# kfkq/DQMC

Hardware: AMD Instinct MI355X
Metric: MC sweeps/sec, 2D Hubbard N=256 Ltau=200 (higher is better)
Workload: dtype f64; 1 GPU; cfg3: 16x16 Hubbard U=8.0 beta=8.0 Ltau=200 n_stab=10 t=1 mu=-0.1; chains_per_gpu=1, n_chains_total=1, parallelism=independent chains, 1 gpu x 1 chain

## Files before the change

dqmc_amd/csrc/common.h:

```cpp
#pragma once

#include <hip/hip_runtime.h>
#include <cstdint>
#include <memory>
#include <string>

struct dqmc_engine;

namespace dq {

constexpr int WAVE = 64;

void set_error(const std::string& msg);
const char* get_error();

#define DQ_HIP(call)                                                                    \
    do {                                                                                \
        hipError_t _e = (call);                                                         \
        if (_e != hipSuccess) {                                                         \
            ::dq::set_error(std::string(#call) + ": " + hipGetErrorString(_e));         \
            return -2;                                              \
        }                                                                               \
    } while (0)

// ... 58 lines not shown
int launch_transpose_scale(CMat in, Mat out, CVec rs, int n, int n_chains, hipStream_t s);
int launch_max_abs_diff(CMat A, CMat B, double* err, long err_stride, int n, int n_chains, hipStream_t s);
int launch_add_scaled_cols(CMat A, CMat B, CVec cs, Mat C, int n, int n_chains, hipStream_t s);
int launch_scale_rows(CMat in, CVec rs, Mat out, int n, int n_chains, hipStream_t s);
struct DevStats { double acc_rate, max_err, sum_err, n_err; long long n_accepted, n_proposed; };
int launch_fold_stats(DevStats* st, const int* acc, long acc_stride, int n_slices, const double* err, long err_stride, int n_err,
                      int n, int nt, int n_chains, hipStream_t s);

struct QrWork {
    double* tau; long tau_stride;
    int* jpvt; long jpvt_stride;
    unsigned long long* sync = nullptr; long sync_stride = 0;
    int* abort_words = nullptr;
    int* info = nullptr;
    double* pw = nullptr; long pw_stride = 0;
    bool pw_two_launch = false;
    int* pivpos = nullptr; long pivpos_stride = 0;
};
bool qr_panel_fused_fits(int n);
bool qr_panel_fused_default(int n);
long qr_panel_work_doubles(int n, bool two_launch);
int launch_qr_panel(Mat A, Mat L, QrWork w, int n, int n_chains, hipStream_t s);
long qrcp_coop_sync_granules(int n);
int qrcp_coop_workgroups(int n, int n_chains);
enum class QrFamily { Panel, ColumnOwner, Cooperative, Streaming };
int launch_to_ldr(QrFamily f, Mat A, Mat L, Vec d, Mat R, QrWork w, int n, int n_chains, hipStream_t s);

int launch_lu_blocked(Mat A, int* perm, long perm_stride, int* rowpos, long rowpos_stride, double* logabsdet, int accumulate_logdet,
                      int* info, int n, int n_chains, hipStream_t s);
int launch_lu_solve(CMat LU, const int* perm, long perm_stride, Mat X, CVec dg, int mode, int n, int n_chains, hipStream_t s);

int launch_tri_solve(CMat R, const int* perm, long perm_stride, Mat X, CVec dg, double* scratch, long scratch_stride, int n, int n_chains, hipStream_t s);

int launch_gj_solve(Mat A, Mat B, Mat X, Mat SA, double* tinv, int* perm, long perm_stride, int* rowpos, long rowpos_stride,
                    double* logabsdet, int accumulate_logdet, int* info, int n, int n_chains, hipStream_t s);

struct UpdateTables {
    double rb[4][3];
    double delta[4][3];
    double ev[4];
    double iev[4];
    double pad[32];
};
struct UpdateDesc {
    Mat G;
    int8_t* fields; long f_stride;
    double* expv; double* invexpv; long v_stride;
    const UpdateTables* tabs;
    const int32_t* perm; const uint8_t* kprop; const double* u; long rs_stride;
    double* Upanel; double* Wpanel; long panel_stride;
    double* Cpanel = nullptr;
    int* state; long state_stride;
    double* prep; long prep_stride;
    Mat GT{nullptr, 0};
    int gt_valid = 0;
    void* slice_sync = nullptr;
    unsigned slice_epoch = 0;
    int slice_absent_tile = -1;
    int slice_absent_l = -1;
    int slice_late_tile = -1, slice_late_us = 0;
    int* info = nullptr;
    int* acc_out; long acc_stride;
    int n, nt;
};
constexpr int UPDATE_KD = 32;

struct SliceSync {
    unsigned long long seq; unsigned int error; unsigned int solo_count; unsigned int pad[12];
// ... 42 lines not shown
```

dqmc_amd/csrc/engine.hip:

```cpp
#include "common.h"
#include "../../include/dqmc_hip.h"

#include <cmath>
#include <cstdlib>
#include <cstring>
#include <map>
#include <memory>
#include <mutex>
#include <vector>

namespace dq {

static thread_local std::string g_err;
void set_error(const std::string& msg) { g_err = msg; }
const char* get_error() { return g_err.c_str(); }

int init_device_kernels(int device) {
    static std::mutex mu; static bool done[64] = {};
    std::lock_guard<std::mutex> lk(mu);
    if (device < 0 || device >= 64) { set_error("device ordinal out of range"); return -1; }
    if (done[device]) return 0;
    DQ_HIP(hipSetDevice(device));
    DQ_TRY(update_init_device()); DQ_TRY(update_sm_init_device()); DQ_TRY(qr_init_device()); DQ_TRY(qr_colown_init_device());
    done[device] = true;
    return 0;
}

struct Switches { bool qr_panel; int qr_panel_fused; bool qr_streaming, walk_submatrix, lu_classic, slice_multikernel; };
static const Switches& switches() {
    static const Switches sw = [] {
        const char* panel = getenv("DQMC_QR_PANEL");
        const char* fused = getenv("DQMC_QR_PANEL_FUSED");
        return Switches{!(panel && atoi(panel) == 0), fused ? (atoi(fused) != 0 ? 1 : 0) : -1, getenv("DQMC_QR_STREAMING") != nullptr, getenv("DQMC_WALK_SUBMATRIX") != nullptr,
                        getenv("DQMC_LU_CLASSIC") != nullptr, getenv("DQMC_SLICE_MULTIKERNEL") != nullptr};
    }();
    return sw;
}

constexpr int GJ_MAX_N = 1024, GJ_MAX_CHAINS = 8;
constexpr int TRI_MAX_N = 640;

static QrFamily pick_qr(int n, int chains, bool allow_panel) {
    const Switches& sw = switches();
    if (sw.qr_streaming) return QrFamily::Streaming;
    if (allow_panel && sw.qr_panel && n >= 64 && n <= 1024 && n % 16 == 0 && chains <= 8) return QrFamily::Panel;
    if (n <= 256) return QrFamily::ColumnOwner;
    return qrcp_coop_workgroups(n, chains) <= 200 ? QrFamily::Cooperative : QrFamily::Streaming;
}

struct KernelPlan {
    QrFamily qr;
    enum class Solve { GaussJordan, BlockedLu } solve;
    enum class Rinv { Blocked, PerColumn } rinv;
    static KernelPlan pick(int n, int chains) {
        return KernelPlan{pick_qr(n, chains, true),
                          n <= GJ_MAX_N && chains <= GJ_MAX_CHAINS && !switches().lu_classic ? Solve::GaussJordan : Solve::BlockedLu,
                          n <= TRI_MAX_N ? Rinv::Blocked : Rinv::PerColumn};
    }
};

static SlicePath pick_slice_path(int n, int chains, bool reserved) {
    const Switches& sw = switches();
    const bool walk = n <= 256;
    if (sw.slice_multikernel) return SlicePath::Pairs;
    if (reserved) return walk && !sw.walk_submatrix ? SlicePath::PersistentWalk : SlicePath::PersistentSubmatrix;
    if (!walk) return SlicePath::Pairs;
// ... 14 lines not shown
    DevPtr<double> L, d, R, X;
    DevPtr<int> jpvt;
    std::unique_ptr<bool[]> tri, xok;
    int alloc(int k, int n_, int C_, bool with_x = false) {
        n = n_; C = C_;
        const size_t nn = (size_t)n * n;
        DQ_TRY(dev_alloc(L, (size_t)k * C * nn)); DQ_TRY(dev_alloc(d, (size_t)k * C * n));
        DQ_TRY(dev_alloc(R, (size_t)k * C * nn)); DQ_TRY(dev_alloc(jpvt, (size_t)k * C * n));
        if (with_x) DQ_TRY(dev_alloc(X, (size_t)k * C * nn));
        tri.reset(new bool[k]()); xok.reset(new bool[k]());
        return 0;
    }
    LdrRef at(int i) const {
        const long nn = (long)n * n;
        LdrRef f{Mat{L.get() + (long)i * C * nn, nn}, Vec{d.get() + (long)i * C * n, (long)n}, Mat{R.get() + (long)i * C * nn, nn},
                 jpvt.get() + (long)i * C * n, &tri[i]};
        if (X) { f.X = Mat{X.get() + (long)i * C * nn, nn}; f.xok = &xok[i]; }
        return f;
    }
};

struct Ctx {
    int n = 0, C = 0, device = 0;
    long nn = 0;
    hipStream_t stream = nullptr;
    static constexpr int NT = 6, NV = 5;
    DevPtr<double> pool;
    DevPtr<double> vpool;
    DevPtr<int> ipool;
    DevPtr<unsigned long long> qsync;
    DevPtr<int> qabort;
    DevPtr<double> tinv;
    DevPtr<double> qpw;
    bool qpw_two_launch = false;
    DevPtr<int> qpivpos;
    DevPtr<double> trinv;
    KernelPlan plan{};

    Mat T(int k) const { return Mat{pool.get() + (long)k * C * nn, nn}; }
    Vec V(int k) const { return Vec{vpool.get() + (long)k * C * n, (long)n}; }
    int* jpvt() const { return ipool.get(); }
    int* lperm() const { return ipool.get() + (long)C * n; }
    int* rowpos() const { return ipool.get() + 2L * C * n; }
    int* info() const { return ipool.get() + 3L * C * n; }

    int init(int n_, int C_, int device_) {
        n = n_; C = C_; device = device_; nn = (long)n * n;
        DQ_HIP(hipSetDevice(device));
        DQ_TRY(init_device_kernels(device));
        DQ_HIP(hipStreamCreateWithFlags(&stream, hipStreamNonBlocking));
        DQ_TRY(dev_alloc(pool, (size_t)NT * C * nn));
        DQ_TRY(dev_alloc(vpool, (size_t)NV * C * n));
        DQ_TRY(dev_alloc(ipool, 3L * C * n + 4));
        plan = KernelPlan::pick(n, C);
        if (plan.qr == QrFamily::Cooperative) { DQ_TRY(dev_alloc(qsync, (size_t)qrcp_coop_sync_granules(n) * C)); DQ_TRY(dev_alloc(qabort, C)); }
        if (plan.qr == QrFamily::Panel) {
            const int fused = switches().qr_panel_fused;
            qpw_two_launch = !(fused < 0 ? qr_panel_fused_default(n) : fused == 1 && qr_panel_fused_fits(n));
            const size_t qpw_count = (size_t)qr_panel_work_doubles(n, qpw_two_launch) * C;
            DQ_TRY(dev_alloc(qpw, qpw_count)); DQ_TRY(dev_alloc(qpivpos, (size_t)n * C));
            DQ_HIP(hipMemsetAsync(qpw.get(), 0, sizeof(double) * qpw_count, stream));
        }
        if (plan.solve == KernelPlan::Solve::GaussJordan) DQ_TRY(dev_alloc(tinv, (size_t)2048 * C));
        if (plan.rinv == KernelPlan::Rinv::Blocked) DQ_TRY(dev_alloc(trinv, (size_t)16 * (n + 16) * C));
        DQ_HIP(hipMemsetAsync(ipool.get(), 0, sizeof(int) * (3L * C * n + 4), stream));
        return 0;
    }
    ~Ctx() { if (stream) (void)hipStreamDestroy(stream); }

    int gemm(CMat A, CMat B, Mat Cm, CVec rs = CVec(), CVec ks = CVec(), CVec cs = CVec(), int transA = 0, int accumulate = 0, Mat CT = Mat{nullptr, 0}) {
        GemmDesc g; g.A = A; g.B = B; g.C = Cm; g.CT = CT; g.rs = rs; g.ks = ks; g.cs = cs; g.n = n; g.transA = transA; g.accumulate = accumulate;
        return launch_gemm(g, C, stream);
    }
    int to_ldr(Mat A, LdrRef out, bool direct = true) {
        const bool keep = direct && out.jpvt != nullptr;
        QrWork w{V(4).p, (long)n, keep ? out.jpvt : jpvt(), (long)n};
        w.sync = qsync.get(); w.sync_stride = qrcp_coop_sync_granules(n); w.abort_words = qabort.get(); w.info = info();
        w.pw = qpw.get(); w.pw_stride = qr_panel_work_doubles(n, qpw_two_launch); w.pw_two_launch = qpw_two_launch; w.pivpos = qpivpos.get(); w.pivpos_stride = n;
        if (out.tri) *out.tri = keep;
        out.touch();
        return launch_to_ldr(plan.qr, A, out.L, out.d, out.R, w, n, C, stream);
    }
    int r_inverse_scaled(LdrRef F, CVec dinv, Mat scratch, Mat lu_scratch, Mat* Xout) {
        const Mat X = F.X.p ? F.X : scratch;
        *Xout = X;
        if (F.xok && *F.xok) return 0;
        if (F.tri && *F.tri && F.jpvt) {
            if (plan.rinv == KernelPlan::Rinv::Blocked) DQ_TRY(launch_tri_solve(F.R, F.jpvt, n, X, dinv, trinv.get(), 16L * (n + 16), n, C, stream));
            else DQ_TRY(launch_lu_solve(F.R, F.jpvt, n, X, dinv, 2, n, C, stream));
        } else {
            DQ_TRY(launch_copy(F.R, lu_scratch, nn, C, stream));
            DQ_TRY(launch_lu_blocked(lu_scratch, lperm(), n, rowpos(), n, nullptr, 0, info(), n, C, stream));
            DQ_TRY(launch_lu_solve(lu_scratch, lperm(), n, X, dinv, 1, n, C, stream));
        }
        if (F.xok) *F.xok = true;
        return 0;
    }
    int mat_mul_ldr(CMat M, LdrRef F, LdrRef out) {
        DQ_TRY(gemm(M, F.L, T(0), CVec(), CVec(), CVec(F.d)));
        LdrRef q{out.L, out.d, T(1)};
        DQ_TRY(to_ldr(T(0), q));
        if (out.tri) *out.tri = false;
        out.touch();
        return gemm(T(1), F.R, out.R);
    }
    int ldr_mul_mat(LdrRef F, CMat M, LdrRef out) {
        DQ_TRY(gemm(F.R, M, T(0), CVec(F.d)));
        LdrRef q{T(1), out.d, out.R, out.jpvt, out.tri};
        q.xok = out.xok;
        DQ_TRY(to_ldr(T(0), q));
        return gemm(F.L, T(1), out.L);
    }
    int ldr_mul_ldr(LdrRef F1, LdrRef F2, LdrRef out) {
        DQ_TRY(gemm(F1.R, F2.L, T(0), CVec(F1.d), CVec(), CVec(F2.d)));
        LdrRef q{T(1), out.d, T(2)};
        DQ_TRY(to_ldr(T(0), q));
        if (out.tri) *out.tri = false;
        out.touch();
        DQ_TRY(gemm(F1.L, T(1), out.L));
        return gemm(T(2), F2.R, out.R);
    }
    int solve(Mat M, Mat RHS, Mat out, double* logdet_acc, Mat* Y) {
        if (plan.solve == KernelPlan::Solve::GaussJordan) {
            DQ_TRY(launch_gj_solve(M, RHS, out, T(5), tinv.get(), lperm(), n, rowpos(), n, logdet_acc, 1, info(), n, C, stream));
            *Y = out; return 0;
        }
        DQ_TRY(launch_lu_blocked(M, lperm(), n, rowpos(), n, logdet_acc, 1, info(), n, C, stream));
        DQ_TRY(launch_lu_solve(M, lperm(), n, RHS, CVec(), 0, n, C, stream));
        *Y = RHS; return 0;
    }
    int inv_I_plus_ldr(LdrRef F, Mat G, double* logdet ) {
        DQ_TRY(launch_split_d(F.d, V(0), V(1), logdet, n, C, stream));
        Mat X; DQ_TRY(r_inverse_scaled(F, V(0), T(1), T(0), &X));
        DQ_TRY(launch_add_scaled_cols(X, F.L, V(1), T(2), n, C, stream));
        DQ_TRY(launch_transpose_scale(T(2), T(3), CVec(), n, C, stream));
        DQ_TRY(launch_transpose_scale(X, T(4), CVec(), n, C, stream));
        Mat Y; DQ_TRY(solve(T(3), T(4), T(0), logdet, &Y));
        return launch_transpose_scale(Y, G, CVec(), n, C, stream);
    }
    int inv_I_plus_ldr_mul_ldr(LdrRef F1, LdrRef F2, Mat G, Mat GT = Mat{nullptr, 0}) {
        DQ_TRY(launch_split_d2(F1.d, V(0), V(1), F2.d, V(2), V(3), n, C, stream));
        Mat X; DQ_TRY(r_inverse_scaled(F2, V(2), T(1), T(0), &X));
        DQ_TRY(gemm(F1.L, X, T(2), V(0), CVec(), CVec(), 1));
        DQ_TRY(gemm(F1.R, F2.L, T(2), V(1), CVec(), V(3), 0, 1));
        DQ_TRY(launch_transpose_scale(F1.L, T(3), V(0), n, C, stream));
        Mat Y; DQ_TRY(solve(T(2), T(3), T(0), nullptr, &Y));
        return gemm(X, Y, G, CVec(), CVec(), CVec(), 0, 0, GT);
    }
    int inv_invldr_plus_ldr(LdrRef F1, LdrRef F2, Mat G, bool negate) {
        DQ_TRY(launch_split_d(F1.d, V(0), V(1), nullptr, n, C, stream));
        DQ_TRY(launch_split_d(F2.d, V(2), V(3), nullptr, n, C, stream));
        Mat X; DQ_TRY(r_inverse_scaled(F2, V(2), T(1), T(0), &X));
        DQ_TRY(gemm(F1.L, X, T(2), V(0), CVec(), CVec(), 1));
        DQ_TRY(gemm(F1.R, F2.L, T(2), V(1), CVec(), V(3), 0, 1));
        DQ_TRY(launch_scale_rows(F1.R, V(1), T(3), n, C, stream));
        Mat Y; DQ_TRY(solve(T(2), T(3), T(0), nullptr, &Y));
        DQ_TRY(gemm(X, Y, G));
// ... 946 lines not shown
```

dqmc_amd/csrc/lu_gj.hip:

```cpp
#include "common.h"
#include "wave.h"
#include <cstdlib>
#include <utility>

namespace dq {

namespace {
constexpr int GJ_NB = 32;
using d4 = __attribute__((ext_vector_type(4))) double;

__device__ __forceinline__ void lds_wait() { asm volatile("s_waitcnt lgkmcnt(0)" ::: "memory"); }

template <int NR, int J>
__device__ __forceinline__ void gj_step(double (&a)[NR][GJ_NB], bool (&live)[NR], int (&mypos)[NR], int& myperm, bool& singular, int lane, int k0) {
    unsigned long long best = 0ULL; int bq = -1;
#pragma unroll
    for (int q = 0; q < NR; ++q) {
        const unsigned long long kq = live[q] ? ((unsigned long long)__double_as_longlong(fabs(a[q][J])) | 1ULL) : 0ULL;
        if (kq > best) { best = kq; bq = q; }
    }
    const unsigned hi = (unsigned)(best >> 32), lo = (unsigned)best;
    const unsigned m1 = wave_max_u32(hi);
    const unsigned m2 = wave_max_u32(hi == m1 ? lo : 0u);
    const unsigned long long winners = __ballot(hi == m1 && lo == m2 && bq >= 0);
// ... 108 lines not shown
            const double s = s0 + s1;
            x[j] = up ? s / T0[sg * (j * 33)] : s;
        }
        double* out = tinv + GJ_NB * GJ_NB + 256 * blk + 16 * c;
#pragma unroll
        for (int j = 0; j < 16; ++j) out[up ? 15 - j : j] = x[j];
    }
}

__device__ __forceinline__ void gj_panel_logdet(double (&LU)[GJ_NB][GJ_NB], double* logabsdet, int accumulate, int* info, int chain, int lane, int nbw, int k0, int s_sing) {
    const double pv = lane < nbw ? fabs(LU[lane][lane]) : 1.0;
    const double ls = wave_sum(log(pv));
    if (lane == 0) {
        if (logabsdet) logabsdet[chain] = ((accumulate || k0 > 0) ? logabsdet[chain] : 0.0) + ls;
        if (info && (s_sing || !(ls == ls))) atomicOr(info, DQ_STATUS_PIVOT);
    }
}
template <int... Js>
__device__ __forceinline__ void gj_tri_steps(double (&x)[16], const double* T0, int sg, int cc, bool up, bool hi, double rd, std::integer_sequence<int, Js...>) {
    auto step = [&](auto jc) {
        constexpr int j = decltype(jc)::value;
        double s0 = (j == cc) ? 1.0 : 0.0, s1 = 0.0;
#pragma unroll
        for (int m = 0; m < j; ++m) {
            const double tt = T0[sg * (j * 32 + m)];
            if (m & 1) s1 = fma(-tt, x[m], s1); else s0 = fma(-tt, x[m], s0);
        }
        const double s = s0 + s1;
        const double r0 = readlane_f64(rd, 15 - j), r1 = readlane_f64(rd, 31 - j);
        x[j] = up ? s * (hi ? r1 : r0) : s;
    };
    (step(std::integral_constant<int, Js>{}), ...);
}
__device__ __forceinline__ void gj_panel_tri_inverses(double (&LU)[GJ_NB][GJ_NB], double* tinv, int lane) {
    const int blk = lane >> 4, c = lane & 15;
    const bool up = blk >= 2;
    const int base = (blk & 1) * 16;
    const double* T0 = &LU[0][0] + (up ? (base + 15) * 33 : base * 33);
    const int sg = up ? -1 : 1;
    const int cc = up ? 15 - c : c;
    const double rd = 1.0 / LU[lane & 31][lane & 31];
    double x[16];
    gj_tri_steps(x, T0, sg, cc, up, (blk & 1) != 0, rd, std::make_integer_sequence<int, 16>{});
    double* out = tinv + GJ_NB * GJ_NB + 256 * blk + 16 * c;
#pragma unroll
    for (int j = 0; j < 16; ++j) out[up ? 15 - j : j] = x[j];
}

#ifdef DQ_GJ_STAMPS
#define GST(i) { unsigned long long t_; asm volatile("s_waitcnt lgkmcnt(0)\n\ts_memtime %0\n\ts_waitcnt lgkmcnt(0)" : "=s"(t_) :: "memory"); gst[i] += t_ - gprev; gprev = t_; }
#define GST_ARGS , unsigned long long (&gst)[8], unsigned long long& gprev
#define GST_PASS , gst, gprev
#else
#define GST(i)
#define GST_ARGS
#define GST_PASS
#endif
template <int J, int NW, int RPL>
__device__ __forceinline__ void gj_step_mw(double (&a)[RPL][GJ_NB], unsigned& live, int (&mypos)[RPL], int& myperm, bool& singular, int lane, int wave, int k0,
                                           double (*slot_row)[NW][GJ_NB + 2], unsigned long long (*slot_key)[(NW + 1) & ~1] GST_ARGS) {
    constexpr int PAR = J & 1;
    constexpr int C0 = J & ~1;
    GST(0)
    double aj = a[0][J]; int bs = 0;
    if (RPL > 1) asm volatile("" : "+v"(aj));
    unsigned long long key = (live & 1u) ? ((unsigned long long)__double_as_longlong(fabs(aj)) | 1ULL) : 0ULL;
#pragma unroll
    for (int q = 1; q < RPL; ++q) {
        double v = a[q][J];
        asm volatile("" : "+v"(v));
        const unsigned long long kq = ((live >> q) & 1u) ? ((unsigned long long)__double_as_longlong(fabs(v)) | 1ULL) : 0ULL;
        if (kq > key) { key = kq; aj = v; bs = q; }
    }
    double rme = __builtin_amdgcn_rcp(aj);
    rme = fma(fma(-aj, rme, 1.0), rme, rme);
    rme = fma(fma(-aj, rme, 1.0), rme, rme);
    const unsigned hi = (unsigned)(key >> 32), lo = (unsigned)key;
// ... 34 lines not shown
    double prow[GJ_NB - C0];
#pragma unroll
    for (int c = C0; c < GJ_NB; c += 2) { const double2 v = *reinterpret_cast<const double2*>(&slot_row[PAR][pw][c]); prow[c - C0] = v.x; prow[c + 1 - C0] = v.y; }
    const double r = slot_row[PAR][pw][GJ_NB];
    GST(5)
    if (lane == J && wave == 0) myperm = pl + 64 * pw + 64 * NW * ps;
    const bool mine = wave == pw && lane == pl;
    singular = singular || !(fabs(prow[J - C0]) > 0.0);
#pragma unroll
    for (int q = 0; q < RPL; ++q) {
        if (mine && ps == q) { live &= ~(1u << q); mypos[q] = k0 + J; }
        const bool lv = (live >> q) & 1u;
        const double l = lv ? a[q][J] * r : 0.0;
        a[q][J] = lv ? l : a[q][J];
#pragma unroll
        for (int c = J + 1; c < GJ_NB; ++c) a[q][c] = fma(-l, prow[c - C0], a[q][c]);
    }
    GST(6)
}
template <int J, int NW, int RPL>
struct GjStepsMW {
    static __device__ __forceinline__ void run(double (&a)[RPL][GJ_NB], unsigned& live, int (&mypos)[RPL], int& myperm, bool& singular, int lane, int wave, int nbw, int k0,
                                               double (*slot_row)[NW][GJ_NB + 2], unsigned long long (*slot_key)[(NW + 1) & ~1] GST_ARGS) {
        if (J < nbw) gj_step_mw<J, NW, RPL>(a, live, mypos, myperm, singular, lane, wave, k0, slot_row, slot_key GST_PASS);
        GjStepsMW<J + 1, NW, RPL>::run(a, live, mypos, myperm, singular, lane, wave, nbw, k0, slot_row, slot_key GST_PASS);
    }
};
template <int NW, int RPL>
struct GjStepsMW<GJ_NB, NW, RPL> {
    static __device__ __forceinline__ void run(double (&)[RPL][GJ_NB], unsigned&, int (&)[RPL], int&, bool&, int, int, int, int, double (*)[NW][GJ_NB + 2],
                                               unsigned long long (*)[(NW + 1) & ~1] GST_ARGS) {}
};
template <int NW, int RPL>
__global__ __launch_bounds__(64 * NW) void gj_panel_mw_kernel(CMat Am, int* rowpos_p, long rowpos_stride, int* perm_p, long perm_stride, double* tinv_p,
                                                          double* logabsdet, int accumulate, int* info, int n, int k0) {
    constexpr int NWK = (NW + 1) & ~1;
    __shared__ __attribute__((aligned(16))) double LU[GJ_NB][GJ_NB];
    __shared__ __attribute__((aligned(16))) double slot_row[2][NW][GJ_NB + 2];
    __shared__ __attribute__((aligned(16))) unsigned long long slot_key[2][NWK];
    __shared__ int s_sing;
    static_assert(RPL <= 4, "two key bits name the slot");
    const int chain = blockIdx.y;
    const double* __restrict__ A = Am.at(chain);
    int* rowpos = rowpos_p + (long)chain * rowpos_stride;
    int* perm = perm_p + (long)chain * perm_stride;
    double* tinv = tinv_p + (long)chain * 2 * GJ_NB * GJ_NB;
    const int t = threadIdx.x, lane = t & 63, wave = t >> 6;
#ifdef DQ_GJ_STAMPS
    unsigned long long gentry;
    asm volatile("s_memtime %0\n\ts_waitcnt lgkmcnt(0)" : "=s"(gentry) :: "memory");
#endif
    const int nbw = min(GJ_NB, n - k0);
    unsigned live = 0u;
    int mypos[RPL], myperm = 0; bool singular = false;
    double a[RPL][GJ_NB];
#pragma unroll
    for (int q = 0; q < RPL; ++q) {
        const int r = t + 64 * NW * q;
        const bool lv = r < n && (k0 == 0 ? true : rowpos[r < n ? r : 0] < 0);
        live |= lv ? (1u << q) : 0u;
        mypos[q] = -1;
#pragma unroll
        for (int c = 0; c < GJ_NB; ++c) a[q][c] = (lv && c < nbw) ? A[r + (long)n * (k0 + c)] : 0.0;
    }
    for (int e = t; e < GJ_NB * GJ_NB; e += blockDim.x) (&LU[0][0])[e] = ((e >> 5) == (e & 31)) ? 1.0 : 0.0;
    if (t == 0) s_sing = 0;
    if (t < 2 * NWK) (&slot_key[0][0])[t] = 0ULL;
    __syncthreads();

#ifdef DQ_GJ_STAMPS
    unsigned long long gst[8] = {0, 0, 0, 0, 0, 0, 0, 0}, gprev, gstart;
    asm volatile("s_waitcnt vmcnt(0)\n\ts_memtime %0\n\ts_waitcnt lgkmcnt(0)" : "=s"(gprev) :: "memory"); gstart = gprev;
#endif
    GjStepsMW<0, NW, RPL>::run(a, live, mypos, myperm, singular, lane, wave, nbw, k0, slot_row, slot_key GST_PASS);
#ifdef DQ_GJ_STAMPS
    if (t == 0 && k0 == 0 && blockIdx.y == 0)
        printf("gj panel k0=0 n=%d, %d waves x %d rows per lane, clocks over %d steps (each segment includes one stamp, ~130): (loop) %llu | search %llu | publish %llu | barrier %llu | keys %llu | row %llu | fma %llu | total %llu\n",
               n, (int)(blockDim.x >> 6), RPL, nbw, gst[0], gst[1], gst[2], gst[3], gst[4], gst[5], gst[6], gprev - gstart);
#endif

    __syncthreads();
#pragma unroll
    for (int q = 0; q < RPL; ++q) {
        const int r = t + 64 * NW * q;
        if (r < n) { if (k0 == 0) rowpos[r] = mypos[q]; else if (mypos[q] >= 0) rowpos[r] = mypos[q]; }
        if (mypos[q] >= 0) {
            double* dst = &LU[mypos[q] - k0][0];
#pragma unroll
            for (int c = 0; c < GJ_NB; c += 2) *reinterpret_cast<double2*>(dst + c) = make_double2(a[q][c], a[q][c + 1]);
        }
    }
    if (wave == 0 && lane < nbw) perm[k0 + lane] = myperm;
    if (singular && lane == 0) s_sing = 1;
    __syncthreads();
    for (int e = t; e < GJ_NB * GJ_NB; e += blockDim.x) tinv[e] = (&LU[0][0])[e];
#ifdef DQ_GJ_STAMPS
    unsigned long long gmid;
    asm volatile("s_waitcnt vmcnt(0)\n\ts_memtime %0\n\ts_waitcnt lgkmcnt(0)" : "=s"(gmid) :: "memory");
#endif
    if (wave == 0) gj_panel_tri_inverses(LU, tinv, lane);
    else if (wave == 1) gj_panel_logdet(LU, logabsdet, accumulate, info, chain, lane, nbw, k0, s_sing);
#ifdef DQ_GJ_STAMPS
    unsigned long long gend;
    asm volatile("s_waitcnt vmcnt(0)\n\ts_memtime %0\n\ts_waitcnt lgkmcnt(0)" : "=s"(gend) :: "memory");
    if (t == 0 && k0 == 0 && blockIdx.y == 0) printf("   prologue %llu | steps %llu | LU hand-over (+ printf) %llu | epilogue %llu\n", gstart - gentry, gprev - gstart, gmid - gprev, gend - gmid);
#endif
}

__global__ __launch_bounds__(256) void gj_update_kernel(Mat Am, Mat Bm, Mat SAm, Mat Xm, const int* rowpos_p, long rowpos_stride,
                                                        const int* perm_p, long perm_stride, const double* tinv_p, int n, int k0, int nA, int nS, int nCA) {
    const int chain = blockIdx.y;
    double* __restrict__ A = Am.at(chain);
    double* __restrict__ B = Bm.at(chain);
    double* __restrict__ SA = SAm.at(chain);
    double* __restrict__ X = Xm.at(chain);
    const int* rowpos = rowpos_p + (long)chain * rowpos_stride;
    const int* perm = perm_p + (long)chain * perm_stride;
    const double* __restrict__ LUg = tinv_p + (long)chain * 2 * GJ_NB * GJ_NB;
    const double* __restrict__ Tinv = LUg + GJ_NB * GJ_NB;
    const int nbw = min(GJ_NB, n - k0);
    const int row_tiles = nA + nS + 1;
    const int rt = blockIdx.x % row_tiles, ct = blockIdx.x / row_tiles;
    const int lane = threadIdx.x & 63, wave = threadIdx.x >> 6;
    const int r16 = lane & 15, kk = lane >> 4;
    const int wr = wave & 1, wc = wave >> 1;
    const bool colA = ct < nCA;
    const int col = (colA ? k0 + nbw + 32 * ct : 32 * (ct - nCA)) + 16 * wc + r16;
    const bool col_ok = col < n;
    const long coff = (long)n * (col_ok ? col : n - 1);
    const double* __restrict__ src12 = colA ? A : B;
    double* __restrict__ dstS = colA ? SA : X;

    double a12[2][4];
#pragma unroll
    for (int h = 0; h < 2; ++h)
#pragma unroll
        for (int s = 0; s < 4; ++s) {
// ... 46 lines not shown
    d4 w = {a12[1][0], a12[1][1], a12[1][2], a12[1][3]};
#pragma unroll
    for (int s = 0; s < 4; ++s) w = __builtin_amdgcn_mfma_f64_16x16x4f64(cl[s], t1[0][s], w, 0, 0, 0);
    t1[1] = zero4;
#pragma unroll
    for (int s = 0; s < 4; ++s) t1[1] = __builtin_amdgcn_mfma_f64_16x16x4f64(lbi[s], w[s], t1[1], 0, 0, 0);
    u[1] = zero4;
#pragma unroll
    for (int s = 0; s < 4; ++s) u[1] = __builtin_amdgcn_mfma_f64_16x16x4f64(ubi[s], t1[1][s], u[1], 0, 0, 0);
    w = t1[0];
#pragma unroll
    for (int s = 0; s < 4; ++s) w = __builtin_amdgcn_mfma_f64_16x16x4f64(cu[s], u[1][s], w, 0, 0, 0);
    u[0] = zero4;
#pragma unroll
    for (int s = 0; s < 4; ++s) u[0] = __builtin_amdgcn_mfma_f64_16x16x4f64(uai[s], w[s], u[0], 0, 0, 0);
    if (writer) {
#pragma unroll
        for (int reg = 0; reg < 4; ++reg) {
            const int i = 16 * wr + kk + 4 * reg;
            if (i < nbw && col_ok) dstS[k0 + i + coff] = u[wr][reg];
        }
        return;
    }
    d4 acc = {0.0, 0.0, 0.0, 0.0};
#pragma unroll
    for (int h = 0; h < 2; ++h)
#pragma unroll
        for (int s = 0; s < 4; ++s) acc = __builtin_amdgcn_mfma_f64_16x16x4f64(mult[h][s], u[h][s], acc, 0, 0, 0);
#pragma unroll
    for (int reg = 0; reg < 4; ++reg)
        if (st_ok[reg]) dst[row0 + kk + 4 * reg + coff] = cold[reg] - acc[reg];
}

int launch_gj_solve(Mat A, Mat B, Mat X, Mat SA, double* tinv, int* perm, long perm_stride, int* rowpos, long rowpos_stride,
                    double* logabsdet, int accumulate_logdet, int* info, int n, int n_chains, hipStream_t s) {
    if (n > 1024) { set_error("gj_solve supports n <= 1024"); return -1; }
    for (int k0 = 0; k0 < n; k0 += GJ_NB) {
        const dim3 pg(1, n_chains);
#define DQ_GJ_PANEL(NW, RPL) hipLaunchKernelGGL((gj_panel_mw_kernel<NW, RPL>), pg, dim3(RPL == 1 ? 64 * ((n + 63) / 64) : 64 * NW), 0, s, CMat(A), rowpos, rowpos_stride, perm, perm_stride, tinv, logabsdet, accumulate_logdet, info, n, k0)
        if (n > 768) DQ_GJ_PANEL(8, 2);
        else if (n > 576) DQ_GJ_PANEL(4, 3);
        else if (n > 512) DQ_GJ_PANEL(3, 3);
        else if (n > 256) DQ_GJ_PANEL(4, 2);
        else if (n > 64) DQ_GJ_PANEL(4, 1);
        else hipLaunchKernelGGL((gj_panel_kernel<1>), pg, dim3(64), 0, s, CMat(A), rowpos, rowpos_stride, perm, perm_stride, tinv, logabsdet, accumulate_logdet, info, n, k0);
        const int nbw = n - k0 < GJ_NB ? n - k0 : GJ_NB;
        const int nA = (n + 31) / 32, nS = k0 / 32;
        const int nCA = (n - k0 - nbw + 31) / 32, nCB = (n + 31) / 32;
        hipLaunchKernelGGL(gj_update_kernel, dim3((nA + nS + 1) * (nCA + nCB), n_chains), dim3(256), 0, s, A, B, SA, X, (const int*)rowpos, rowpos_stride,
                           (const int*)perm, perm_stride, (const double*)tinv, n, k0, nA, nS, nCA);
    }
#undef DQ_GJ_PANEL
    DQ_HIP(hipGetLastError());
    return 0;
}

}
```

Measured before the change: 13.02 sweeps/s.

## Fuse Gauss-Jordan panel factorization into the update kernel with redundant per-block panels

Adds a fused gj_step_kernel that has every update workgroup redundantly factor the 32-column panel, compute the triangular inverses in shared memory, and then apply the trailing update. This halves the launches per block step and removes the serial single-workgroup panel kernel and its global hand-off of tinv. Row positions ping-pong between two buffers so that blocks reading old positions do not race with the writer. It is enabled by default for 128 < n <= 256, which covers N=256. The cost is redundant panel work in every block and higher shared-memory and register pressure.

Result: faster. 13.19 sweeps/s (median of 6 runs) (+1.3%).

```diff
diff --git a/dqmc_amd/csrc/common.h b/dqmc_amd/csrc/common.h
--- a/dqmc_amd/csrc/common.h
+++ b/dqmc_amd/csrc/common.h
@@ -114,8 +114,10 @@
 
 int launch_tri_solve(CMat R, const int* perm, long perm_stride, Mat X, CVec dg, double* scratch, long scratch_stride, int n, int n_chains, hipStream_t s);
 
-int launch_gj_solve(Mat A, Mat B, Mat X, Mat SA, double* tinv, int* perm, long perm_stride, int* rowpos, long rowpos_stride,
-                    double* logabsdet, int accumulate_logdet, int* info, int n, int n_chains, hipStream_t s);
+bool gj_fused_fits(int n);
+bool gj_fused_default(int n);
+int launch_gj_solve(Mat A, Mat B, Mat X, Mat SA, double* tinv, int* perm, long perm_stride, int* rowpos, int* rowpos_alt, long rowpos_stride,
+                    double* logabsdet, int accumulate_logdet, int* info, int n, int n_chains, bool fused, hipStream_t s);
 
 struct UpdateTables {
     double rb[4][3];
diff --git a/dqmc_amd/csrc/engine.hip b/dqmc_amd/csrc/engine.hip
--- a/dqmc_amd/csrc/engine.hip
+++ b/dqmc_amd/csrc/engine.hip
@@ -26,12 +26,13 @@
     return 0;
 }
 
-struct Switches { bool qr_panel; int qr_panel_fused; bool qr_streaming, walk_submatrix, lu_classic, slice_multikernel; };
+struct Switches { bool qr_panel; int qr_panel_fused, gj_fused; bool qr_streaming, walk_submatrix, lu_classic, slice_multikernel; };
 static const Switches& switches() {
     static const Switches sw = [] {
         const char* panel = getenv("DQMC_QR_PANEL");
         const char* fused = getenv("DQMC_QR_PANEL_FUSED");
-        return Switches{!(panel && atoi(panel) == 0), fused ? (atoi(fused) != 0 ? 1 : 0) : -1, getenv("DQMC_QR_STREAMING") != nullptr, getenv("DQMC_WALK_SUBMATRIX") != nullptr,
+        const char* gj = getenv("DQMC_GJ_FUSED");
+        return Switches{!(panel && atoi(panel) == 0), fused ? (atoi(fused) != 0 ? 1 : 0) : -1, gj ? (atoi(gj) != 0 ? 1 : 0) : -1, getenv("DQMC_QR_STREAMING") != nullptr, getenv("DQMC_WALK_SUBMATRIX") != nullptr,
                         getenv("DQMC_LU_CLASSIC") != nullptr, getenv("DQMC_SLICE_MULTIKERNEL") != nullptr};
     }();
     return sw;
@@ -112,6 +113,7 @@
     DevPtr<int> qabort;
     DevPtr<double> tinv;
     DevPtr<double> qpw;
+    bool gj_fused = false;
     bool qpw_two_launch = false;
     DevPtr<int> qpivpos;
     DevPtr<double> trinv;
@@ -122,7 +124,8 @@
     int* jpvt() const { return ipool.get(); }
     int* lperm() const { return ipool.get() + (long)C * n; }
     int* rowpos() const { return ipool.get() + 2L * C * n; }
-    int* info() const { return ipool.get() + 3L * C * n; }
+    int* rowpos_alt() const { return ipool.get() + 3L * C * n; }
+    int* info() const { return ipool.get() + 4L * C * n; }
 
     int init(int n_, int C_, int device_) {
         n = n_; C = C_; device = device_; nn = (long)n * n;
@@ -131,7 +134,7 @@
         DQ_HIP(hipStreamCreateWithFlags(&stream, hipStreamNonBlocking));
         DQ_TRY(dev_alloc(pool, (size_t)NT * C * nn));
         DQ_TRY(dev_alloc(vpool, (size_t)NV * C * n));
-        DQ_TRY(dev_alloc(ipool, 3L * C * n + 4));
+        DQ_TRY(dev_alloc(ipool, 4L * C * n + 4));
         plan = KernelPlan::pick(n, C);
         if (plan.qr == QrFamily::Cooperative) { DQ_TRY(dev_alloc(qsync, (size_t)qrcp_coop_sync_granules(n) * C)); DQ_TRY(dev_alloc(qabort, C)); }
         if (plan.qr == QrFamily::Panel) {
@@ -141,9 +144,13 @@
             DQ_TRY(dev_alloc(qpw, qpw_count)); DQ_TRY(dev_alloc(qpivpos, (size_t)n * C));
             DQ_HIP(hipMemsetAsync(qpw.get(), 0, sizeof(double) * qpw_count, stream));
         }
-        if (plan.solve == KernelPlan::Solve::GaussJordan) DQ_TRY(dev_alloc(tinv, (size_t)2048 * C));
+        if (plan.solve == KernelPlan::Solve::GaussJordan) {
+            DQ_TRY(dev_alloc(tinv, (size_t)2048 * C));
+            const int fused = switches().gj_fused;
+            gj_fused = fused < 0 ? gj_fused_default(n) : fused == 1 && gj_fused_fits(n);
+        }
         if (plan.rinv == KernelPlan::Rinv::Blocked) DQ_TRY(dev_alloc(trinv, (size_t)16 * (n + 16) * C));
-        DQ_HIP(hipMemsetAsync(ipool.get(), 0, sizeof(int) * (3L * C * n + 4), stream));
+        DQ_HIP(hipMemsetAsync(ipool.get(), 0, sizeof(int) * (4L * C * n + 4), stream));
         return 0;
     }
     ~Ctx() { if (stream) (void)hipStreamDestroy(stream); }
@@ -202,7 +209,7 @@
     }
     int solve(Mat M, Mat RHS, Mat out, double* logdet_acc, Mat* Y) {
         if (plan.solve == KernelPlan::Solve::GaussJordan) {
-            DQ_TRY(launch_gj_solve(M, RHS, out, T(5), tinv.get(), lperm(), n, rowpos(), n, logdet_acc, 1, info(), n, C, stream));
+            DQ_TRY(launch_gj_solve(M, RHS, out, T(5), tinv.get(), lperm(), n, rowpos(), rowpos_alt(), n, logdet_acc, 1, info(), n, C, gj_fused, stream));
             *Y = out; return 0;
         }
         DQ_TRY(launch_lu_blocked(M, lperm(), n, rowpos(), n, logdet_acc, 1, info(), n, C, stream));
diff --git a/dqmc_amd/csrc/lu_gj.hip b/dqmc_amd/csrc/lu_gj.hip
--- a/dqmc_amd/csrc/lu_gj.hip
+++ b/dqmc_amd/csrc/lu_gj.hip
@@ -164,7 +164,7 @@
     };
     (step(std::integral_constant<int, Js>{}), ...);
 }
-__device__ __forceinline__ void gj_panel_tri_inverses(double (&LU)[GJ_NB][GJ_NB], double* tinv, int lane) {
+__device__ __forceinline__ void gj_panel_tri_inverses(double (&LU)[GJ_NB][GJ_NB], double* inv, int lane) {
     const int blk = lane >> 4, c = lane & 15;
     const bool up = blk >= 2;
     const int base = (blk & 1) * 16;
@@ -174,7 +174,7 @@
     const double rd = 1.0 / LU[lane & 31][lane & 31];
     double x[16];
     gj_tri_steps(x, T0, sg, cc, up, (blk & 1) != 0, rd, std::make_integer_sequence<int, 16>{});
-    double* out = tinv + GJ_NB * GJ_NB + 256 * blk + 16 * c;
+    double* out = inv + 256 * blk + 16 * c;
 #pragma unroll
     for (int j = 0; j < 16; ++j) out[up ? 15 - j : j] = x[j];
 }
@@ -275,14 +275,91 @@
                                                unsigned long long (*)[(NW + 1) & ~1] GST_ARGS) {}
 };
 template <int NW, int RPL>
+struct GjPanelShared {
+    double LU[GJ_NB][GJ_NB];
+    double slot_row[2][NW][GJ_NB + 2];
+    unsigned long long slot_key[2][(NW + 1) & ~1];
+    int s_sing;
+};
+template <int NW, int RPL, bool CLAMPED>
+__device__ __forceinline__ void gj_panel_load(const double* __restrict__ A, const int* rowpos, int n, int k0, int nbw, int t, double (&a)[RPL][GJ_NB], unsigned& live,
+                                              int (&oldpos)[RPL]) {
+    live = 0u;
+#pragma unroll
+    for (int q = 0; q < RPL; ++q) {
+        const int r = t + 64 * NW * q;
+        const int rc = r < n ? r : 0;
+        if (CLAMPED) {
+            double v[GJ_NB];
+#pragma unroll
+            for (int c = 0; c < GJ_NB; ++c) v[c] = A[rc + (long)n * (k0 + (c < nbw ? c : 0))];
+            oldpos[q] = k0 == 0 ? -1 : rowpos[rc];
+            const bool lv = r < n && oldpos[q] < 0;
+            live |= lv ? (1u << q) : 0u;
+#pragma unroll
+            for (int c = 0; c < GJ_NB; ++c) a[q][c] = (lv && c < nbw) ? v[c] : 0.0;
+        } else {
+            oldpos[q] = k0 == 0 ? -1 : rowpos[rc];
+            const bool lv = r < n && oldpos[q] < 0;
+            live |= lv ? (1u << q) : 0u;
+#pragma unroll
+            for (int c = 0; c < GJ_NB; ++c) a[q][c] = (lv && c < nbw) ? A[r + (long)n * (k0 + c)] : 0.0;
+        }
+    }
+}
+template <int NW, int RPL>
+__device__ __forceinline__ void gj_panel_factor(GjPanelShared<NW, RPL>& sh, double (&a)[RPL][GJ_NB], unsigned& live, int (&mypos)[RPL], int& myperm, int t, int nbw, int k0
+#ifdef DQ_GJ_STAMPS
+                                                , unsigned long long& gstart, unsigned long long& gsteps_end
+#endif
+                                                ) {
+    constexpr int NWK = (NW + 1) & ~1;
+    static_assert(RPL <= 4, "two key bits name the slot");
+    const int lane = t & 63, wave = t >> 6;
+    bool singular = false;
+    myperm = 0;
+#pragma unroll
+    for (int q = 0; q < RPL; ++q) mypos[q] = -1;
+    for (int e = t; e < GJ_NB * GJ_NB; e += blockDim.x) (&sh.LU[0][0])[e] = ((e >> 5) == (e & 31)) ? 1.0 : 0.0;
+    if (t == 0) sh.s_sing = 0;
+    if (t < 2 * NWK) (&sh.slot_key[0][0])[t] = 0ULL;
+    lds_wait();
+    __builtin_amdgcn_s_barrier();
+    asm volatile("" ::: "memory");
+
+#ifdef DQ_GJ_STAMPS
+    unsigned long long gst[8] = {0, 0, 0, 0, 0, 0, 0, 0}, gprev;
+    asm volatile("s_waitcnt vmcnt(0)\n\ts_memtime %0\n\ts_waitcnt lgkmcnt(0)" : "=s"(gprev) :: "memory"); gstart = gprev;
+#endif
+    GjStepsMW<0, NW, RPL>::run(a, live, mypos, myperm, singular, lane, wave, nbw, k0, sh.slot_row, sh.slot_key GST_PASS);
+#ifdef DQ_GJ_STAMPS
+    gsteps_end = gprev;
+    if (t == 0 && k0 == 0 && blockIdx.x == 0 && blockIdx.y == 0)
+        printf("gj panel k0=0 grid.x=%d, %d waves x %d rows per lane, clocks over %d steps (each segment includes one stamp, ~130): (loop) %llu | search %llu | publish %llu | barrier %llu | keys %llu | row %llu | fma %llu | total %llu\n",
+               (int)gridDim.x, (int)(blockDim.x >> 6), RPL, nbw, gst[0], gst[1], gst[2], gst[3], gst[4], gst[5], gst[6], gprev - gstart);
+#endif
+
+    lds_wait();
+    __builtin_amdgcn_s_barrier();
+    asm volatile("" ::: "memory");
+#pragma unroll
+    for (int q = 0; q < RPL; ++q) {
+        if (mypos[q] >= 0) {
+            double* dst = &sh.LU[mypos[q] - k0][0];
+#pragma unroll
+            for (int c = 0; c < GJ_NB; c += 2) *reinterpret_cast<double2*>(dst + c) = make_double2(a[q][c], a[q][c + 1]);
+        }
+    }
+    if (singular && lane == 0) sh.s_sing = 1;
+}
+#ifdef DQ_GJ_STAMPS
+#define GJ_STAMP_VM(x) asm volatile("s_waitcnt vmcnt(0)\n\ts_memtime %0\n\ts_waitcnt lgkmcnt(0)" : "=s"(x) :: "memory")
+#endif
+
+template <int NW, int RPL>
 __global__ __launch_bounds__(64 * NW) void gj_panel_mw_kernel(CMat Am, int* rowpos_p, long rowpos_stride, int* perm_p, long perm_stride, double* tinv_p,
                                                           double* logabsdet, int accumulate, int* info, int n, int k0) {
-    constexpr int NWK = (NW + 1) & ~1;
-    __shared__ __attribute__((aligned(16))) double LU[GJ_NB][GJ_NB];
-    __shared__ __attribute__((aligned(16))) double slot_row[2][NW][GJ_NB + 2];
-    __shared__ __attribute__((aligned(16))) unsigned long long slot_key[2][NWK];
-    __shared__ int s_sing;
-    static_assert(RPL <= 4, "two key bits name the slot");
+    __shared__ __attribute__((aligned(16))) GjPanelShared<NW, RPL> sh;
     const int chain = blockIdx.y;
     const double* __restrict__ A = Am.at(chain);
     int* rowpos = rowpos_p + (long)chain * rowpos_stride;
@@ -290,62 +367,36 @@
     double* tinv = tinv_p + (long)chain * 2 * GJ_NB * GJ_NB;
     const int t = threadIdx.x, lane = t & 63, wave = t >> 6;
 #ifdef DQ_GJ_STAMPS
-    unsigned long long gentry;
+    unsigned long long gentry, gstart, gprev;
     asm volatile("s_memtime %0\n\ts_waitcnt lgkmcnt(0)" : "=s"(gentry) :: "memory");
 #endif
     const int nbw = min(GJ_NB, n - k0);
-    unsigned live = 0u;
-    int mypos[RPL], myperm = 0; bool singular = false;
+    unsigned live;
+    int oldpos[RPL], mypos[RPL], myperm;
     double a[RPL][GJ_NB];
-#pragma unroll
-    for (int q = 0; q < RPL; ++q) {
-        const int r = t + 64 * NW * q;
-        const bool lv = r < n && (k0 == 0 ? true : rowpos[r < n ? r : 0] < 0);
-        live |= lv ? (1u << q) : 0u;
-        mypos[q] = -1;
-#pragma unroll
-        for (int c = 0; c < GJ_NB; ++c) a[q][c] = (lv && c < nbw) ? A[r + (long)n * (k0 + c)] : 0.0;
-    }
-    for (int e = t; e < GJ_NB * GJ_NB; e += blockDim.x) (&LU[0][0])[e] = ((e >> 5) == (e & 31)) ? 1.0 : 0.0;
-    if (t == 0) s_sing = 0;
-    if (t < 2 * NWK) (&slot_key[0][0])[t] = 0ULL;
-    __syncthreads();
-
-#ifdef DQ_GJ_STAMPS
-    unsigned long long gst[8] = {0, 0, 0, 0, 0, 0, 0, 0}, gprev, gstart;
-    asm volatile("s_waitcnt vmcnt(0)\n\ts_memtime %0\n\ts_waitcnt lgkmcnt(0)" : "=s"(gprev) :: "memory"); gstart = gprev;
-#endif
-    GjStepsMW<0, NW, RPL>::run(a, live, mypos, myperm, singular, lane, wave, nbw, k0, slot_row, slot_key GST_PASS);
-#ifdef DQ_GJ_STAMPS
-    if (t == 0 && k0 == 0 && blockIdx.y == 0)
-        printf("gj panel k0=0 n=%d, %d waves x %d rows per lane, clocks over %d steps (each segment includes one stamp, ~130): (loop) %llu | search %llu | publish %llu | barrier %llu | keys %llu | row %llu | fma %llu | total %llu\n",
-               n, (int)(blockDim.x >> 6), RPL, nbw, gst[0], gst[1], gst[2], gst[3], gst[4], gst[5], gst[6], gprev - gstart);
-#endif
-
-    __syncthreads();
+    gj_panel_load<NW, RPL, false>(A, rowpos, n, k0, nbw, t, a, live, oldpos);
+#ifdef DQ_GJ_STAMPS
+    gj_panel_factor<NW, RPL>(sh, a, live, mypos, myperm, t, nbw, k0, gstart, gprev);
+#else
+    gj_panel_factor<NW, RPL>(sh, a, live, mypos, myperm, t, nbw, k0);
+#endif
 #pragma unroll
     for (int q = 0; q < RPL; ++q) {
         const int r = t + 64 * NW * q;
         if (r < n) { if (k0 == 0) rowpos[r] = mypos[q]; else if (mypos[q] >= 0) rowpos[r] = mypos[q]; }
-        if (mypos[q] >= 0) {
-            double* dst = &LU[mypos[q] - k0][0];
-#pragma unroll
-            for (int c = 0; c < GJ_NB; c += 2) *reinterpret_cast<double2*>(dst + c) = make_double2(a[q][c], a[q][c + 1]);
-        }
     }
     if (wave == 0 && lane < nbw) perm[k0 + lane] = myperm;
-    if (singular && lane == 0) s_sing = 1;
     __syncthreads();
-    for (int e = t; e < GJ_NB * GJ_NB; e += blockDim.x) tinv[e] = (&LU[0][0])[e];
+    for (int e = t; e < GJ_NB * GJ_NB; e += blockDim.x) tinv[e] = (&sh.LU[0][0])[e];
 #ifdef DQ_GJ_STAMPS
     unsigned long long gmid;
-    asm volatile("s_waitcnt vmcnt(0)\n\ts_memtime %0\n\ts_waitcnt lgkmcnt(0)" : "=s"(gmid) :: "memory");
-#endif
-    if (wave == 0) gj_panel_tri_inverses(LU, tinv, lane);
-    else if (wave == 1) gj_panel_logdet(LU, logabsdet, accumulate, info, chain, lane, nbw, k0, s_sing);
+    GJ_STAMP_VM(gmid);
+#endif
+    if (wave == 0) gj_panel_tri_inverses(sh.LU, tinv + GJ_NB * GJ_NB, lane);
+    else if (wave == 1) gj_panel_logdet(sh.LU, logabsdet, accumulate, info, chain, lane, nbw, k0, sh.s_sing);
 #ifdef DQ_GJ_STAMPS
     unsigned long long gend;
-    asm volatile("s_waitcnt vmcnt(0)\n\ts_memtime %0\n\ts_waitcnt lgkmcnt(0)" : "=s"(gend) :: "memory");
+    GJ_STAMP_VM(gend);
     if (t == 0 && k0 == 0 && blockIdx.y == 0) printf("   prologue %llu | steps %llu | LU hand-over (+ printf) %llu | epilogue %llu\n", gstart - gentry, gprev - gstart, gmid - gprev, gend - gmid);
 #endif
 }
@@ -458,9 +509,181 @@
         if (st_ok[reg]) dst[row0 + kk + 4 * reg + coff] = cold[reg] - acc[reg];
 }
 
-int launch_gj_solve(Mat A, Mat B, Mat X, Mat SA, double* tinv, int* perm, long perm_stride, int* rowpos, long rowpos_stride,
-                    double* logabsdet, int accumulate_logdet, int* info, int n, int n_chains, hipStream_t s) {
+template <int NW, int RPL>
+__global__ __launch_bounds__(64 * NW) void gj_step_kernel(Mat Am, Mat Bm, Mat SAm, Mat Xm, const int* rowpos_old_p, int* rowpos_new_p, long rowpos_stride,
+                                                          double* logabsdet, int accumulate, int* info, int n, int k0, int nA, int nS, int nCA) {
+    static_assert(NW == 4, "the update's 2 x 2 waves are the panel's");
+    __shared__ __attribute__((aligned(16))) GjPanelShared<NW, RPL> sh;
+    __shared__ __attribute__((aligned(16))) double s_inv[4 * 256];
+    __shared__ int s_rowpos[64 * NW * RPL];
+    __shared__ int s_perm[GJ_NB];
+    const int chain = blockIdx.y;
+    double* __restrict__ A = Am.at(chain);
+    double* __restrict__ B = Bm.at(chain);
+    double* __restrict__ SA = SAm.at(chain);
+    double* __restrict__ X = Xm.at(chain);
+    const int* rowpos_old = rowpos_old_p + (long)chain * rowpos_stride;
+    int* rowpos_new = rowpos_new_p + (long)chain * rowpos_stride;
+    const int t = threadIdx.x, lane = t & 63, wave = t >> 6;
+#ifdef DQ_GJ_STAMPS
+    unsigned long long gentry, gstart, gprev;
+    asm volatile("s_memtime %0\n\ts_waitcnt lgkmcnt(0)" : "=s"(gentry) :: "memory");
+#endif
+    const int nbw = min(GJ_NB, n - k0);
+
+    unsigned live;
+    int oldpos[RPL], mypos[RPL], myperm;
+    double a[RPL][GJ_NB];
+    gj_panel_load<NW, RPL, true>(A, rowpos_old, n, k0, nbw, t, a, live, oldpos);
+
+    const int row_tiles = nA + nS + 1;
+    const int rt = blockIdx.x % row_tiles, ct = blockIdx.x / row_tiles;
+    const int r16 = lane & 15, kk = lane >> 4;
+    const int wr = wave & 1, wc = wave >> 1;
+    const bool colA = ct < nCA;
+    const int col = (colA ? k0 + nbw + 32 * ct : 32 * (ct - nCA)) + 16 * wc + r16;
+    const bool col_ok = col < n;
+    const long coff = (long)n * (col_ok ? col : n - 1);
+    const double* __restrict__ src12 = colA ? A : B;
+    double* __restrict__ dstS = colA ? SA : X;
+    const bool writer = rt == nA + nS;
+    const bool rowS = rt >= nA;
+    const int row0 = (rowS ? 32 * (rt - nA) : 32 * rt) + 16 * wr;
+    const int rowlim = rowS ? k0 : n;
+    const double* __restrict__ msrc = rowS ? SA : A;
+    double* __restrict__ dst = rowS ? dstS : (colA ? A : B);
+    double mult[2][4];
+    double cold[4];
+    {
+        const int mrow = max(min(row0 + r16, rowlim - 1), 0);
+#pragma unroll
+        for (int h = 0; h < 2; ++h)
+#pragma unroll
+            for (int s = 0; s < 4; ++s) {
+                const int k = 16 * h + kk + 4 * s;
+                const double v = msrc[mrow + (long)n * (k0 + (k < nbw ? k : 0))];
+                mult[h][s] = k < nbw ? v : 0.0;
+            }
+#pragma unroll
+        for (int reg = 0; reg < 4; ++reg) cold[reg] = dst[max(min(row0 + kk + 4 * reg, rowlim - 1), 0) + coff];
+    }
+
+#ifdef DQ_GJ_STAMPS
+    gj_panel_factor<NW, RPL>(sh, a, live, mypos, myperm, t, nbw, k0, gstart, gprev);
+#else
+    gj_panel_factor<NW, RPL>(sh, a, live, mypos, myperm, t, nbw, k0);
+#endif
+#pragma unroll
+    for (int q = 0; q < RPL; ++q) {
+        const int r = t + 64 * NW * q;
+        const int np = mypos[q] >= 0 ? mypos[q] : oldpos[q];
+        s_rowpos[r] = np;
+        if (blockIdx.x == 0 && r < n) rowpos_new[r] = np;
+    }
+    if (wave == 0 && lane < GJ_NB) s_perm[lane] = lane < nbw ? myperm : 0;
+    __syncthreads();
+#ifdef DQ_GJ_STAMPS
+    unsigned long long gmid, ginv, ggather;
+    GJ_STAMP_VM(gmid);
+#endif
+
+    double a12[2][4];
+#pragma unroll
+    for (int h = 0; h < 2; ++h)
+#pragma unroll
+        for (int s = 0; s < 4; ++s) {
+            const int k = 16 * h + 4 * s + kk;
+            const double v = src12[s_perm[k < nbw ? k : 0] + coff];
+            a12[h][s] = (k < nbw && col_ok) ? v : 0.0;
+        }
+    bool st_ok[4];
+#pragma unroll
+    for (int reg = 0; reg < 4; ++reg) {
+        const int r = row0 + kk + 4 * reg;
+        st_ok[reg] = !writer && col_ok && r < rowlim && (rowS || s_rowpos[max(min(r, rowlim - 1), 0)] < 0);
+    }
+    if (wave == 0) gj_panel_tri_inverses(sh.LU, s_inv, lane);
+    else if (wave == 1 && blockIdx.x == 0) gj_panel_logdet(sh.LU, logabsdet, accumulate, info, chain, lane, nbw, k0, sh.s_sing);
+#ifdef DQ_GJ_STAMPS
+    asm volatile("s_waitcnt lgkmcnt(0)\n\ts_memtime %0\n\ts_waitcnt lgkmcnt(0)" : "=s"(ginv) :: "memory");
+#endif
+    __syncthreads();
+#ifdef DQ_GJ_STAMPS
+    GJ_STAMP_VM(ggather);
+#endif
+
+    const double* LUs = &sh.LU[0][0];
+    double lai[4], lbi[4], uai[4], ubi[4], cl[4], cu[4];
+#pragma unroll
+    for (int s = 0; s < 4; ++s) {
+        const int k = 4 * s + kk;
+        lai[s] = s_inv[0 * 256 + r16 + 16 * k]; lbi[s] = s_inv[1 * 256 + r16 + 16 * k];
+        uai[s] = s_inv[2 * 256 + r16 + 16 * k]; ubi[s] = s_inv[3 * 256 + r16 + 16 * k];
+        cl[s] = -LUs[(16 + r16) * 32 + k];
+        cu[s] = -LUs[r16 * 32 + 16 + k];
+    }
+    const d4 zero4 = {0.0, 0.0, 0.0, 0.0};
+    d4 t1[2], u[2];
+    t1[0] = zero4;
+#pragma unroll
+    for (int s = 0; s < 4; ++s) t1[0] = __builtin_amdgcn_mfma_f64_16x16x4f64(lai[s], a12[0][s], t1[0], 0, 0, 0);
+    d4 w = {a12[1][0], a12[1][1], a12[1][2], a12[1][3]};
+#pragma unroll
+    for (int s = 0; s < 4; ++s) w = __builtin_amdgcn_mfma_f64_16x16x4f64(cl[s], t1[0][s], w, 0, 0, 0);
+    t1[1] = zero4;
+#pragma unroll
+    for (int s = 0; s < 4; ++s) t1[1] = __builtin_amdgcn_mfma_f64_16x16x4f64(lbi[s], w[s], t1[1], 0, 0, 0);
+    u[1] = zero4;
+#pragma unroll
+    for (int s = 0; s < 4; ++s) u[1] = __builtin_amdgcn_mfma_f64_16x16x4f64(ubi[s], t1[1][s], u[1], 0, 0, 0);
+    w = t1[0];
+#pragma unroll
+    for (int s = 0; s < 4; ++s) w = __builtin_amdgcn_mfma_f64_16x16x4f64(cu[s], u[1][s], w, 0, 0, 0);
+    u[0] = zero4;
+#pragma unroll
+    for (int s = 0; s < 4; ++s) u[0] = __builtin_amdgcn_mfma_f64_16x16x4f64(uai[s], w[s], u[0], 0, 0, 0);
+    if (writer) {
+#pragma unroll
+        for (int reg = 0; reg < 4; ++reg) {
+            const int i = 16 * wr + kk + 4 * reg;
+            if (i < nbw && col_ok) dstS[k0 + i + coff] = u[wr][reg];
+        }
+    } else {
+        d4 acc = {0.0, 0.0, 0.0, 0.0};
+#pragma unroll
+        for (int h = 0; h < 2; ++h)
+#pragma unroll
+            for (int s = 0; s < 4; ++s) acc = __builtin_amdgcn_mfma_f64_16x16x4f64(mult[h][s], u[h][s], acc, 0, 0, 0);
+#pragma unroll
+        for (int reg = 0; reg < 4; ++reg)
+            if (st_ok[reg]) dst[row0 + kk + 4 * reg + coff] = cold[reg] - acc[reg];
+    }
+#ifdef DQ_GJ_STAMPS
+    unsigned long long gend;
+    GJ_STAMP_VM(gend);
+    if (t == 0 && k0 == 0 && blockIdx.x == 0 && blockIdx.y == 0)
+        printf("   fused step: prologue %llu | chain %llu | deposit (+ printf) %llu | inverses (wave 0) %llu | gather wait %llu | update %llu\n", gstart - gentry, gprev - gstart,
+               gmid - gprev, ginv - gmid, ggather - ginv, gend - ggather);
+#endif
+}
+bool gj_fused_fits(int n) { return n > 64 && n <= 256; }
+bool gj_fused_default(int n) { return n > 128 && n <= 256; }
+
+int launch_gj_solve(Mat A, Mat B, Mat X, Mat SA, double* tinv, int* perm, long perm_stride, int* rowpos, int* rowpos_alt, long rowpos_stride,
+                    double* logabsdet, int accumulate_logdet, int* info, int n, int n_chains, bool fused, hipStream_t s) {
     if (n > 1024) { set_error("gj_solve supports n <= 1024"); return -1; }
+    if (fused && rowpos_alt && gj_fused_fits(n)) {
+        int p = 0;
+        for (int k0 = 0; k0 < n; k0 += GJ_NB, ++p) {
+            const int nbw = n - k0 < GJ_NB ? n - k0 : GJ_NB;
+            const int nA = (n + 31) / 32, nS = k0 / 32;
+            const int nCA = (n - k0 - nbw + 31) / 32, nCB = (n + 31) / 32;
+            hipLaunchKernelGGL((gj_step_kernel<4, 1>), dim3((nA + nS + 1) * (nCA + nCB), n_chains), dim3(256), 0, s, A, B, SA, X, (const int*)((p & 1) ? rowpos_alt : rowpos),
+                               (p & 1) ? rowpos : rowpos_alt, rowpos_stride, logabsdet, accumulate_logdet, info, n, k0, nA, nS, nCA);
+        }
+        DQ_HIP(hipGetLastError());
+        return 0;
+    }
     for (int k0 = 0; k0 < n; k0 += GJ_NB) {
         const dim3 pg(1, n_chains);
 #define DQ_GJ_PANEL(NW, RPL) hipLaunchKernelGGL((gj_panel_mw_kernel<NW, RPL>), pg, dim3(RPL == 1 ? 64 * ((n + 63) / 64) : 64 * NW), 0, s, CMat(A), rowpos, rowpos_stride, perm, perm_stride, tinv, logabsdet, accumulate_logdet, info, n, k0)
```
